# thetisproject/thetis

Measured on AMD Instinct MI355X. Metric: DG element-updates/sec, 2D SWE DG-P1 SSPRK33, higher is better.
Workload: dtype f64

## Files before the change

thetis_amd/csrc/swe2d_api_fuse.hip:

```cpp
#include "swe2d_handle.h"
#include "swe2d_fuse.h"
#include "swe2d_tiles.h"

#include <type_traits>

namespace swe2d_impl {

namespace {
template <bool... B, class F> auto pick_instance(F f) { return f(std::bool_constant<B>{}...); }
template <bool... B, class F, class... Rest> auto pick_instance(F f, bool b, Rest... rest)
{
    return b ? pick_instance<B..., true>(f, rest...) : pick_instance<B..., false>(f, rest...);
}

const TileSpec kPairTiles{3, 1, SWE_FUSE_WG, SWE_FUSE_INNER, SWE_FUSE_RING, SWE_FUSE_MAX_OUT, false};
const TileSpec kQuadPairTiles{4, 1, SWE_FUSE_WG, SWE_QFUSE_INNER, SWE_QFUSE_RING, SWE_QFUSE_MAX_OUT, false};
const TileSpec kTripleTiles{3, 2, SWE_FUSE_WG, SWE_FUSE_WG, -1, SWE_FUSE3_MAX_OUT, true};

int build_table(Handle *h, const TileSpec &spec, const std::vector<int> &order, const std::vector<unsigned char> &start, TileTable &t)
{
    const int n = h->n_cells;
    std::string err;
    if (build_tiles(h->h_nbr.data(), h->stride, n, (int)order.size() == n ? order.data() : nullptr,
                    (int)start.size() == n ? start.data() : nullptr, spec, t, err))
        return fail(h, SWE2D_ERR_UNSUPPORTED, err);
    return SWE2D_OK;
}

std::vector<int> tile_records(const TileTable &t, int nfacets)
{
    std::vector<int> rec;
    for (size_t i = 0; i < t.cell.size(); i++) {
        const unsigned *w = &t.facet[i*nfacets];
        rec.push_back(t.cell[i]);
        rec.push_back((int)(w[0] | (w[1] << SWE_FUSE_FBITS) | (w[2] << (2*SWE_FUSE_FBITS))));
        if (nfacets == 4) { rec.push_back((int)w[3]); rec.push_back(0); }
    }
    return rec;
}

int upload_tiles(Handle *h, TileSet &ts, const std::vector<int> &rec, const std::vector<int> &counts, const TileTable &t)
{
    HIP_TRY(h, hipMalloc(&ts.tile, rec.size()*sizeof(int)));
    HIP_TRY(h, hipMalloc(&ts.counts, counts.size()*sizeof(int)));
    HIP_TRY(h, hipMemcpy(ts.tile, rec.data(), rec.size()*sizeof(int), hipMemcpyHostToDevice));
    HIP_TRY(h, hipMemcpy(ts.counts, counts.data(), counts.size()*sizeof(int), hipMemcpyHostToDevice));
    ts.n_tiles = (int)t.n_inner.size();
    ts.ring[0] = t.ring[0]; ts.ring[1] = t.ring[1];
    return SWE2D_OK;
}
}

void free_tiles(TileSet &ts)
{
    if (ts.tile) (void)hipFree(ts.tile);
    if (ts.counts) (void)hipFree(ts.counts);
    ts = TileSet();
}

int fuse12_build(Handle *h)
{
    TileSet &ts = pair_tiles(h);
    if (ts.tile || h->fuse_state == -1 || stream_capturing(h)) return SWE2D_OK;
    TileTable t;
    if (int rc = build_table(h, h->npc == 4 ? kQuadPairTiles : kPairTiles, h->fuse_order, {}, t)) return rc;
    if (!fuse12_tiles_pay(h, (int)t.n_inner.size())) { h->fuse_state = -1; return SWE2D_OK; }
    return upload_tiles(h, ts, tile_records(t, h->npc), t.n_inner, t);
}

template <class Args>
static int launch_pair(Handle *h, void (*kern)(const Args), int cell_end)
{
    const TileSet &ts = pair_tiles(h);
    if (!ts.tile) return fail(h, SWE2D_ERR_UNSUPPORTED, "fused stage pair: no tile tables");
    Args q;
    fill_stage_args(h, q.st, 0, 0, 2, 0.0, 1.0, kBeta[0], 0, h->n_owned);
    q.st.idxc = h->opt[SWE2D_OPT_COMPACT_IDX] == 0 ? nullptr : h->idxc;
    q.tile = static_cast<decltype(q.tile)>(ts.tile);
    q.n_inner = ts.counts;
    q.n_tiles = ts.n_tiles;
    q.cell_end = cell_end;
    q.beta1 = kBeta[0];
    q.a0_2 = kAlpha0[1]; q.a1_2 = kAlphaIn[1]; q.beta2 = kBeta[1];
    q.out = h->state[2];
    const int grid = ((ts.n_tiles + 7)/8)*8;
    SWE_CHK_SYNC(h->stream);
    hipLaunchKernelGGL(kern, dim3(grid), dim3(SWE_FUSE_WG), 0, h->stream, q);
    HIP_TRY(h, hipGetLastError());
    stage_written(h, false, true);
    return SWE2D_OK;
}

int launch_fuse12(Handle *h, int cell_end)
{
    const bool nl = h->par.use_nonlinear_equations != 0, lf = h->par.use_lax_friedrichs_velocity != 0;
    if (h->npc == 4)
        return launch_pair(h, pick_instance([](auto a, auto b, auto c, auto d) -> void (*)(const SweFuseQuadArgs) {
                               return swe_fuse12_quad_kernel<a.value, b.value, c.value, d.value>; }, nl, lf, has_sources(h), h->affine), cell_end);
    return launch_pair(h, pick_instance([](auto a, auto b, auto c) -> void (*)(const SweFuseArgs) {
                           return swe_fuse12_kernel<a.value, b.value, c.value>; }, nl, lf, has_sources(h)), cell_end);
}

int fuse123_build(Handle *h)
{
    if (h->fuse3.tile || stream_capturing(h)) return SWE2D_OK;
    TileTable t;
    if (int rc = build_table(h, kTripleTiles, (int)h->fuse3_order.size() == h->n_cells ? h->fuse3_order : h->fuse_order, h->fuse3_start, t)) return rc;
    std::vector<int> counts;
    for (size_t i = 0; i < t.n_inner.size(); i++) { counts.push_back(t.n_inner[i]); counts.push_back(t.n_mid[i] | (t.rot[i] << 16)); }
    return upload_tiles(h, h->fuse3, tile_records(t, 3), counts, t);
}

int launch_fuse123(Handle *h, int cell_end)
{
    if (int rc = capture_parity_check(h)) return rc;
    if (int rc = fuse123_build(h)) return rc;
    if (!h->fuse3.tile) return fail(h, SWE2D_ERR_UNSUPPORTED, "fused stages: no tile tables (not built inside a stream capture)");
    SweFuse3Args q;
    fill_stage_args(h, q.st, 0, 0, 1, 0.0, 1.0, kBeta[0], 0, h->n_owned);
    q.st.idxc = h->opt[SWE2D_OPT_COMPACT_IDX] == 0 ? nullptr : h->idxc;
    q.tile = static_cast<const int2 *>(h->fuse3.tile);
    q.counts = reinterpret_cast<const int2 *>(h->fuse3.counts);
    q.n_tiles = h->fuse3.n_tiles;
    q.cell_end = cell_end;
    for (int s = 0; s < 3; s++) { q.a0[s] = s ? kAlpha0[s] : 0.0; q.a1[s] = s ? kAlphaIn[s] : 1.0; q.beta[s] = kBeta[s]; }
    q.out = h->state[1];
    auto kern = pick_instance([](auto a, auto b, auto c) -> void (*)(const SweFuse3Args) { return swe_fuse123_kernel<a.value, b.value, c.value>; },
                              h->par.use_nonlinear_equations != 0, h->par.use_lax_friedrichs_velocity != 0, has_sources(h));
    const int grid = ((h->fuse3.n_tiles + 7)/8)*8;
    SWE_CHK_SYNC(h->stream);
    hipLaunchKernelGGL(kern, dim3(grid), dim3(SWE_FUSE_WG), 0, h->stream, q);
    HIP_TRY(h, hipGetLastError());
    swap_state_buffers(h);
    unsigned long long id = 0;
    if (stream_capturing(h, &id)) {
        if (id != h->capture_id) { h->capture_id = id; h->capture_swaps = 0; }
        h->capture_swaps++;
    }
    return SWE2D_OK;
}

int capture_parity_check(Handle *h)
{
    if (h->capture_swaps == 0 && h->capture_odd == 0) return SWE2D_OK;
    unsigned long long id = 0;
    const bool capturing = stream_capturing(h, &id);
    if (h->capture_swaps) {
        if (capturing && id == h->capture_id) return SWE2D_OK;
        if (h->capture_swaps & 1) { swap_state_buffers(h); h->capture_odd++; }
        h->capture_swaps = 0;
    }
    if (capturing || h->capture_odd == 0) return SWE2D_OK;
    const int odd = h->capture_odd;
    h->capture_odd = 0;
    return fail(h, SWE2D_ERR_UNSUPPORTED, std::to_string(odd) + " stream capture(s) recorded an odd number of swe2d_solve_step_cells launches: "
                "such a graph ends on the other state buffer than it began on and cannot be replayed (the state is the one from before the "
                "capture); capture an even number per sequence");
}

}

static int checked_tile_order(Handle *h, const int32_t *cells, std::vector<int> &order)
{
    std::vector<char> seen((size_t)h->n_cells, 0);
    for (int i = 0; cells && i < h->n_cells; i++) {
        if (cells[i] < 0 || cells[i] >= h->n_cells || seen[cells[i]]) return fail(h, SWE2D_ERR_INVALID_ARGUMENT, "fused stages: the tile order is not a permutation of the cells");
        seen[cells[i]] = 1;
    }
    if (cells) order.assign(cells, cells + h->n_cells);
    return SWE2D_OK;
}

extern "C" {

int swe2d_fused_set_order(swe2d_handle *hh, const int32_t *cells_in_tile_order)
{
    Handle *h = H(hh);
    if (!h) return SWE2D_ERR_INVALID_ARGUMENT;
    HIP_TRY(h, hipSetDevice(h->device));
    std::vector<int> order;
    if (int rc = checked_tile_order(h, cells_in_tile_order, order)) return rc;
    HIP_TRY(h, hipStreamSynchronize(h->stream));
    for (TileSet *ts : {&h->fuse, &h->fuseq, &h->fuse3}) free_tiles(*ts);
    if (h->fuse_state == -1) h->fuse_state = 0;
    h->fuse_order.swap(order);
    return SWE2D_OK;
}

int swe2d_fused_set_triple_tiles(swe2d_handle *hh, const int32_t *cells_in_tile_order, const int32_t *tile_starts, int32_t n_starts)
{
    Handle *h = H(hh);
    if (!h) return SWE2D_ERR_INVALID_ARGUMENT;
    HIP_TRY(h, hipSetDevice(h->device));
    std::vector<int> order;
    std::vector<unsigned char> start;
    if (int rc = checked_tile_order(h, cells_in_tile_order, order)) return rc;
    if (n_starts < 0 || (n_starts > 0 && !tile_starts)) return fail(h, SWE2D_ERR_INVALID_ARGUMENT, "fused stages: tile starts");
    if (n_starts > 0) {
        start.assign((size_t)h->n_cells, 0);
        for (int i = 0; i < n_starts; i++) {
            if (tile_starts[i] < 0 || tile_starts[i] >= h->n_cells) return fail(h, SWE2D_ERR_INVALID_ARGUMENT, "fused stages: a tile start outside the cells");
            start[tile_starts[i]] = 1;
        }
    }
    HIP_TRY(h, hipStreamSynchronize(h->stream));
// ... 50 lines not shown
```

thetis_amd/csrc/swe2d_flow.h:

```cpp
#pragma once
#include "swe2d_kernels.h"
#include "swe2d_p2p.h"

#ifndef SWE_FLOW_OCCUPANCY
#define SWE_FLOW_OCCUPANCY __attribute__((amdgpu_waves_per_eu(2, 2)))
#endif
#define SWE_FLOW_MAX_STAGES 384
#define SWE_FLOW_MAX_CYCLES 64
#ifndef SWE_FLOW_FLAG_STRIDE
#define SWE_FLOW_FLAG_STRIDE 16
#endif
#define SWE_FLOW_SLOT_BYTES 128
#define SWE_FLOW_DIV6(t_) ((int)(((unsigned)(t_)*43691u) >> 18))
#ifndef SWE_FLOW_POLL_SLEEP
#define SWE_FLOW_POLL_SLEEP 2
#endif
#ifndef SWE_FLOW_NTR_SRC
#define SWE_FLOW_NTR_SRC 3
#endif
#ifndef SWE_FLOW_WALLFAST_SRC
#define SWE_FLOW_WALLFAST_SRC true
#endif
#ifndef SWE_FLOW_RX
#define SWE_FLOW_RX 3
// ... 37 lines not shown
    const int4 *xo4;
    const int2 *xo2;
    const int2 *xblk;
    const int *xsrc;
    void *ex;
    unsigned parity_bytes;
    int n_blocks;
    int n_stages;
    int cell_end[SWE_FLOW_MAX_STAGES];
    double a0[3], a1[3], beta[3];
    unsigned long long timeout_ticks;
    int n_cycles, stages_per_cycle;
    const int2 *xsend;
    const int *xrecv;
    unsigned *xtick;
    SweP2pCounters *xctr;
    int x_n_peers;
    int x_off[SWE_P2P_MAX_PEERS];
    void *x_rdata[SWE_P2P_MAX_PEERS];
    unsigned x_rbytes[SWE_P2P_MAX_PEERS];
    unsigned x_rslot[SWE_P2P_MAX_PEERS];
    void *x_zone;
    unsigned x_zbytes, x_slot;
    unsigned long long x_timeout;
};

__device__ __forceinline__ unsigned swe_flow_check_word(unsigned lo, unsigned hi, unsigned tag) { return tag ^ lo ^ hi; }
#ifdef SWE_FLOW_TEAR
__device__ int swe_flow_tear[4] = {-1, 0, 1, 0};
__device__ __forceinline__ void swe_flow_put_torn(__amdgpu_buffer_rsrc_t r, unsigned off, swe_u32x4 g, int aux_sys, int ticks)
{
    const swe_u32x2 hi2 = {g.z, g.w}, lo2 = {g.x, g.y};
    if (aux_sys) __builtin_amdgcn_raw_buffer_store_b64(hi2, r, off + 8u, 0, 17); else __builtin_amdgcn_raw_buffer_store_b64(hi2, r, off + 8u, 0, 16);
    asm volatile("s_waitcnt vmcnt(0)" ::: "memory");
    const unsigned long long t0 = wall_clock64();
    while (wall_clock64() - t0 < (unsigned long long)ticks) __builtin_amdgcn_s_sleep(16);
    if (aux_sys) __builtin_amdgcn_raw_buffer_store_b64(lo2, r, off, 0, 17); else __builtin_amdgcn_raw_buffer_store_b64(lo2, r, off, 0, 16);
}
#define SWE_FLOW_TORN(lb_, pc_, sys_) ((swe_flow_tear[0] == (lb_) || swe_flow_tear[0] == -2) && swe_flow_tear[1] > 0 \
                                       && ((pc_) % (swe_flow_tear[2] < 1 ? 1 : swe_flow_tear[2])) == 0 && (!(sys_) || swe_flow_tear[3]))
#endif
__device__ __forceinline__ void swe_flow_put(__amdgpu_buffer_rsrc_t r, unsigned off, double x, unsigned tag, bool torn = false)
{
    const swe_u32x2 xb = __builtin_bit_cast(swe_u32x2, x);
    const swe_u32x4 g = {xb.x, xb.y, tag, swe_flow_check_word(xb.x, xb.y, tag)};
#ifdef SWE_FLOW_TEAR
    if (torn) { swe_flow_put_torn(r, off, g, 0, swe_flow_tear[1]); return; }
#endif
    (void)torn;
    __builtin_amdgcn_raw_buffer_store_b128(g, r, off, 0, 16);
}
__device__ __forceinline__ swe_u32x4 swe_flow_get(__amdgpu_buffer_rsrc_t r, unsigned off)
{
    return __builtin_amdgcn_raw_buffer_load_b128(r, off, 0, 16);
}
__device__ __forceinline__ void swe_flow_put_sys(__amdgpu_buffer_rsrc_t r, unsigned off, double x, unsigned tag, bool torn = false)
{
    const swe_u32x2 xb = __builtin_bit_cast(swe_u32x2, x);
    const swe_u32x4 g = {xb.x, xb.y, tag, swe_flow_check_word(xb.x, xb.y, tag)};
#ifdef SWE_FLOW_TEAR
    if (torn) { swe_flow_put_torn(r, off, g, 1, swe_flow_tear[1]); return; }
#endif
    (void)torn;
    __builtin_amdgcn_raw_buffer_store_b128(g, r, off, 0, 17);
}
__device__ __forceinline__ swe_u32x4 swe_flow_get_sys(__amdgpu_buffer_rsrc_t r, unsigned off)
{
    return __builtin_amdgcn_raw_buffer_load_b128(r, off, 0, 17);
}
__device__ __forceinline__ double swe_flow_val(swe_u32x4 g)
{
    const swe_u32x2 xb = {g.x, g.y};
    return __builtin_bit_cast(double, xb);
}
__device__ __forceinline__ bool swe_flow_arrived(swe_u32x4 g, unsigned need)
{
#ifdef SWE_FLOW_NOCHECK
    return (int)(g.z - need) >= 0;
#else
    return (int)(g.z - need) >= 0 && g.w == swe_flow_check_word(g.x, g.y, g.z);
#endif
}

template <bool NONLIN, bool LF, bool SRC, int NTR, bool WD = false, int XG = SWE_FLOW_XG, int PLANE = SWE_BLOCK, int NLDS = SWE_FLOW_LDS_DOUBLES,
          int GEOM = SWE_GEOM_COMPUTE>
__device__ __forceinline__ void swe_flow_rhs_facets(const SweStageArgs &p, int k, const double u[3], const double v[3], const double e[3],
                                                    const double h[3], const double *lds, const unsigned tr[3][NTR], int bmarkers,
                                                    const double nx[3], const double ny[3], double twoA, double bu[3], double bv[3],
                                                    double be[3], const double *Dn = nullptr, const double *al = nullptr, double *geo = nullptr)
{
#pragma clang fp contract(off)
#pragma unroll
    for (int f = 0; f < 3; f++) {
        const int a = f, b = (f + 1) % 3;
        const unsigned ab0 = tr[f][0] & 0xffffu, aa0 = tr[f][0] >> 16;
        const unsigned step = ab0 >= (unsigned)XG ? 1u : (unsigned)(3*PLANE);
        const unsigned ab1 = NTR == 3 ? tr[f][NTR - 2] & 0xffffu : ab0 + step, aa1 = NTR == 3 ? tr[f][NTR - 2] >> 16 : aa0 + step;
        const unsigned ab2 = NTR == 3 ? tr[f][NTR - 1] & 0xffffu : ab0 + 2u*step, aa2 = NTR == 3 ? tr[f][NTR - 1] >> 16 : aa0 + 2u*step;
        const double unb = lds[SWE_LDSI(ab0, NLDS)], una = lds[SWE_LDSI(aa0, NLDS)];
        const double vnb = lds[SWE_LDSI(ab1, NLDS)], vna = lds[SWE_LDSI(aa1, NLDS)];
        const double enb = lds[SWE_LDSI(ab2, NLDS)], ena = lds[SWE_LDSI(aa2, NLDS)];
        double Lf, rLf;
        if constexpr (GEOM == SWE_GEOM_STORED) { Lf = geo[f*PLANE]; rLf = geo[(3 + f)*PLANE]; }
        else swe_tri_facet_len(nx[f], ny[f], Lf, rLf);
        if constexpr (GEOM == SWE_GEOM_KEEP) { geo[f*PLANE] = Lf; geo[(3 + f)*PLANE] = rLf; }
        swe_tri_facet<NONLIN, LF, WD>(p.g, p.sigma_lf, ((bmarkers >> (8*f)) & 0xff) != 0, u[a], u[b], v[a], v[b], e[a], e[b], h[a], h[b],
                                      WD ? Dn[a] : 0.0, WD ? Dn[b] : 0.0, WD ? al[a] : 0.0, WD ? al[b] : 0.0, una, unb, vna, vnb, ena, enb,
                                      nx[f], ny[f], Lf, rLf, bu[a], bu[b], bv[a], bv[b], be[a], be[b]);
    }
    if (SRC) {
        double H[3], gxs[3], gys[3];
        swe_tri_depths<NONLIN, WD>(h, e, Dn, H);
        swe_tri_grad(nx, ny, gxs, gys);
        swe_source_terms(p, k, p.stride, twoA, u, v, H, gxs, gys, bu, bv, be);
    }
}

#ifdef SWE_WAVE_TIMING
#ifndef SWE_FLOW_TS_STAGE
#define SWE_FLOW_TS_STAGE 7
#endif
#define SWE_FT(i) do { if (s == SWE_FLOW_TS_STAGE && lane == 0 && lb < SWE_WT_MAX) swe_wave_ts[i][lb] = wall_clock64(); } while (0)
#else
#define SWE_FT(i)
#endif


template <bool NONLIN, bool LF, bool SRC, bool FX, int POLL = 6, bool WD = false>
__global__ __launch_bounds__(SWE_BLOCK) SWE_FLOW_OCCUPANCY void swe_flow_kernel(const SweFlowArgs q)
{
#pragma clang fp contract(off)
    __shared__ double lds[SWE_FLOW_LDS_DOUBLES];
    __shared__ int xsrc[SWE_FLOW_MAX_RIM];
    __shared__ int lact[SWE_BLOCK];
    __shared__ unsigned lrec[SWE_BLOCK];
    __shared__ int lpeer[SWE_BLOCK];
    __shared__ unsigned char lpub[SWE_FLOW_MAX_RIM];
    __shared__ double lu0[9][SWE_BLOCK];
    const SweStageArgs &p = q.st;
    const int lb = swe_logical_block(blockIdx.x, gridDim.x);
    if (lb >= q.n_blocks) return;
    const int lane = (int)threadIdx.x;
    const int kcode = q.fcell[lb*SWE_BLOCK + lane];
    const bool real = kcode >= 0;
    const int k = real ? kcode : -1 - kcode;
    const size_t S = p.stride;
    const unsigned S8 = (unsigned)S*8u;
    unsigned *const myflag = q.flag + (size_t)lb*SWE_FLOW_FLAG_STRIDE;
    const unsigned base = *myflag;
    const unsigned fin = base + (unsigned)q.n_stages;
    if (!FX && !__any(real && k < q.cell_end[0])) {
        if (lane == 0) *myflag = fin;
        return;
    }
    const unsigned k8 = (unsigned)k*8u;
    const __amdgpu_buffer_rsrc_t rex = __builtin_amdgcn_make_buffer_rsrc(q.ex, 0, 3*q.parity_bytes, 0x00020000);
    const int2 myslots = q.xblk[lb];
    const int nrim = myslots.y;
    for (int i = lane; i < nrim; i += SWE_BLOCK) xsrc[SWE_LDSI(i, SWE_FLOW_MAX_RIM)] = q.xsrc[myslots.x + i];

    int bmarkers, bkind1 = 0;
    constexpr int NTR = WD ? 1 : SWE_FLOW_NTR_SRC;
    unsigned tr[3][NTR];
    int xown[3];
    double h[3], nx[3], ny[3], al[3] = {0.0, 0.0, 0.0};
    double u[3], v[3], e[3];
    {
        const int4 q4 = p.idx4[k];
        const int2 q2 = p.idx2[k];
        const int4 x4 = q.xo4[lb*SWE_BLOCK + lane];
        const int2 x2 = q.xo2[lb*SWE_BLOCK + lane];
        const int nb[3] = {q4.x, q4.y, q4.z};
        const int vid[3] = {q4.w, q2.x, q2.y};
        const int xin[3] = {x4.w, x2.x, x2.y};
        xown[0] = x4.x; xown[1] = x4.y; xown[2] = x4.z;
        bmarkers = (nb[0] < 0 ? -nb[0] : 0) | (nb[1] < 0 ? (-nb[1]) << 8 : 0) | (nb[2] < 0 ? (-nb[2]) << 16 : 0);
        if (bmarkers != 0) {
            const int m1 = (bmarkers & 0xff) ? (bmarkers & 0xff) : ((bmarkers & 0xff00) ? ((bmarkers >> 8) & 0xff) : (bmarkers >> 16));
            bkind1 = m1 < SWE_MAX_MARKERS ? p.bc.kind[m1] : 0;
        }
        const swe_rsrc_t gu = swe_rsrc(q.buf[0]), gv = swe_rsrc(q.buf[0] + 3*S), ge = swe_rsrc(q.buf[0] + 6*S);
#pragma unroll
        for (int i = 0; i < 3; i++) {
            u[i] = swe_ld(gu, k8, i*S8);
// ... 437 lines not shown
```

thetis_amd/csrc/swe2d_fuse.h:

```cpp
#pragma once
#include "swe2d_kernels.h"
#include "swe2d_flow.h"

#ifndef SWE_FUSE_WG
#define SWE_FUSE_WG 256
#endif
#ifndef SWE_FUSE_MIN_WG
#define SWE_FUSE_MIN_WG 3
#endif
#ifndef SWE_FUSE_INNER
#define SWE_FUSE_INNER 192
#endif
#define SWE_FUSE_FBITS 10
#define SWE_FUSE_RING (SWE_FUSE_WG - SWE_FUSE_INNER)
#define SWE_FUSE_XG (9*SWE_FUSE_WG)
#define SWE_FUSE_MAX_OUT (2*SWE_FUSE_RING)
#define SWE_FUSE_LDS (SWE_FUSE_XG + 6*SWE_FUSE_MAX_OUT)

struct SweFuseArgs {
    SweStageArgs st;
    const int2 *tile;
    const int *n_inner;
    int n_tiles;
    int cell_end;
// ... 79 lines not shown
#pragma unroll
        for (int f = 0; f < 3; f++) {
            if (outside[f]) {
                const unsigned at = ((unsigned)tl.y >> (SWE_FUSE_FBITS*f)) & 0x1ffu;
#pragma unroll
                for (int j = 0; j < 6; j++) lds[SWE_LDSI(SWE_FUSE_XG + 6*at + j, SWE_FUSE_LDS)] = r0[f][j];
            }
        }
    }
    __syncthreads();
    double o1u[3], o1v[3], o1e[3];
    double twoA = 0.0;
    if (real) {
        twoA = fma(nx[0], ny[1], -(ny[0]*nx[1]));
        double bu[3], bv[3], be[3], wu[3], wv[3], we[3];
        double H[3];
        swe_tri_depths<NONLIN, false>(h, e, nullptr, H);
        swe_tri_cell<NONLIN>(p.g, u, v, e, H, nx, ny, bu, bv, be);
        swe_flow_rhs_facets<NONLIN, LF, SRC, 1, false, SWE_FUSE_XG, SWE_FUSE_WG, SWE_FUSE_LDS>(p, k, u, v, e, h, lds, tr, bmarkers, nx, ny, twoA, bu, bv, be);
#pragma unroll
        for (int i = 0; i < 3; i++) { wu[i] = 1.0*u[i]; wv[i] = 1.0*v[i]; we[i] = 1.0*e[i]; }
        swe_tri_finish<NONLIN, LF, false, true>(p, k, q.beta1, twoA, u, v, e, h, nullptr, nullptr, nx, ny, bmarkers, bkind1, bu, bv, be,
                                                wu, wv, we, true, o1u, o1v, o1e);
    }
    __syncthreads();
    if (real) {
#pragma unroll
        for (int i = 0; i < 3; i++) { lds[i*SWE_FUSE_WG + lane] = o1u[i]; lds[(3 + i)*SWE_FUSE_WG + lane] = o1v[i]; lds[(6 + i)*SWE_FUSE_WG + lane] = o1e[i]; }
    }
    const bool act2 = lane < n_inner && k < q.cell_end;
    if (act2) {
#pragma unroll
        for (int i = 0; i < 3; i++) {
            lw[i][lane] = fma(q.a0_2, u[i], q.a1_2*o1u[i]);
            lw[3 + i][lane] = fma(q.a0_2, v[i], q.a1_2*o1v[i]);
            lw[6 + i][lane] = fma(q.a0_2, e[i], q.a1_2*o1e[i]);
        }
    }
    __syncthreads();
    if (act2) {
#pragma unroll
        for (int i = 0; i < 3; i++) asm volatile("" : "+v"(nx[i]), "+v"(ny[i]), "+v"(h[i]));
#pragma unroll
        for (int f = 0; f < 3; f++) asm volatile("" : "+v"(tr[f][0]));
        asm volatile("" : "+v"(bmarkers), "+v"(twoA));
        double bu[3], bv[3], be[3], wu[3], wv[3], we[3], ou[3], ov[3], oe[3];
        double H[3];
        swe_tri_depths<NONLIN, false>(h, o1e, nullptr, H);
        swe_tri_cell<NONLIN>(p.g, o1u, o1v, o1e, H, nx, ny, bu, bv, be);
        swe_flow_rhs_facets<NONLIN, LF, SRC, 1, false, SWE_FUSE_XG, SWE_FUSE_WG, SWE_FUSE_LDS>(p, k, o1u, o1v, o1e, h, lds, tr, bmarkers, nx, ny, twoA, bu, bv, be);
#pragma unroll
        for (int i = 0; i < 3; i++) { wu[i] = lw[i][lane]; wv[i] = lw[3 + i][lane]; we[i] = lw[6 + i][lane]; }
        swe_tri_finish<NONLIN, LF, false, true>(p, k, q.beta2, twoA, o1u, o1v, o1e, h, nullptr, nullptr, nx, ny, bmarkers, bkind1, bu, bv, be,
                                                wu, wv, we, true, ou, ov, oe);
        const swe_rsrc_t gou = swe_rsrc(q.out), gov = swe_rsrc(q.out + 3*S), goe = swe_rsrc(q.out + 6*S);
#pragma unroll
        for (int i = 0; i < 3; i++) {
            swe_st(gou, k8, i*S8, ou[i]);
            swe_st(gov, k8, i*S8, ov[i]);
            swe_st(goe, k8, i*S8, oe[i]);
        }
    }
}

#ifndef SWE_FUSE3_MAX_OUT
#define SWE_FUSE3_MAX_OUT 224
#endif
#ifndef SWE_FUSE3_GEOM
#define SWE_FUSE3_GEOM 1
#endif
#define SWE_FUSE3_NGEO 7
#define SWE_FUSE3_GEO (18*SWE_FUSE_WG)
#define SWE_FUSE3_XG (SWE_FUSE3_GEOM ? 9*SWE_FUSE_WG : 18*SWE_FUSE_WG)
#define SWE_FUSE3_LDS (SWE_FUSE3_GEOM ? SWE_FUSE3_GEO + SWE_FUSE3_NGEO*SWE_FUSE_WG : SWE_FUSE3_XG + 6*SWE_FUSE3_MAX_OUT)
static_assert(6*SWE_FUSE3_MAX_OUT <= 9*SWE_FUSE_WG, "the staging area must fit P1");
#ifndef SWE_FUSE3_SRC_MIN_WG
#define SWE_FUSE3_SRC_MIN_WG 2
#endif

struct SweFuse3Args {
    SweStageArgs st;
    const int2 *tile;
    const int2 *counts;
    int n_tiles;
    int cell_end;
    double a0[3], a1[3], beta[3];
    double *out;
};

template <bool NONLIN, bool LF, bool SRC = false>
__global__ __launch_bounds__(SWE_FUSE_WG, SRC ? SWE_FUSE3_SRC_MIN_WG : SWE_FUSE_MIN_WG) void swe_fuse123_kernel(const SweFuse3Args q)
{
#pragma clang fp contract(off)
    __shared__ double lds[SWE_FUSE3_LDS];
    const SweStageArgs &p = q.st;
    const int tile = swe_logical_block(blockIdx.x, gridDim.x);
    if (tile >= q.n_tiles) return;
    const int lane = (int)threadIdx.x;
    const int2 tl = q.tile[(size_t)tile*SWE_FUSE_WG + lane];
    const bool real = tl.x >= 0;
    const int k = real ? tl.x : 0;
    const int2 cnt = q.counts[tile];
    const int n_inner = cnt.x, n_mid = cnt.y & 0xffff, rot64 = (cnt.y >> 16) << 6;
    const size_t S = p.stride;
    const unsigned S8 = (unsigned)S*8u, k8 = (unsigned)k*8u;
    double *const P1 = lds + 9*SWE_FUSE_WG;
#ifdef SWE_WAVE_TIMING
    int wt_bodies = __any(real) ? 1 : 0;
#endif

    int bmarkers = 0, bkind1 = 0;
    unsigned tr[3][1];
    double h[3], nx[3], ny[3], u[3], v[3], e[3];
    if (real) {
        int nb[3], vid[3];
        swe_conn_load(p.idxc, p.idx4, p.idx2, k, nb, vid);
        bmarkers = (nb[0] < 0 ? -nb[0] : 0) | (nb[1] < 0 ? (-nb[1]) << 8 : 0) | (nb[2] < 0 ? (-nb[2]) << 16 : 0);
        if (bmarkers != 0) {
            const int m1 = (bmarkers & 0xff) ? (bmarkers & 0xff) : ((bmarkers & 0xff00) ? ((bmarkers >> 8) & 0xff) : (bmarkers >> 16));
            bkind1 = m1 < SWE_MAX_MARKERS ? p.bc.kind[m1] : 0;
        }
        const swe_rsrc_t gu = swe_rsrc(p.uin), gv = swe_rsrc(p.uin + 3*S), ge = swe_rsrc(p.uin + 6*S);
#pragma unroll
        for (int i = 0; i < 3; i++) {
            u[i] = swe_ld(gu, k8, i*S8);
            v[i] = swe_ld(gv, k8, i*S8);
            e[i] = swe_ld(ge, k8, i*S8);
        }
        double r0[3][6];
        bool outside[3];
#pragma unroll
        for (int f = 0; f < 3; f++) {
            const int nbf = nb[f];
            const unsigned w = ((unsigned)tl.y >> (SWE_FUSE_FBITS*f)) & 0x3ffu;
            outside[f] = (w & 0x200u) != 0u;
            const unsigned at = w & 0x1ffu;
            const int f2 = nbf >= 0 ? (nbf & 3) : f, f2a = f2 == 2 ? 0 : f2 + 1;
            {
                const unsigned ab = outside[f] ? (unsigned)(SWE_FUSE3_XG + 6*at) : (unsigned)(f2*SWE_FUSE_WG + at);
                const unsigned aa = outside[f] ? (unsigned)(SWE_FUSE3_XG + 6*at + 3) : (unsigned)(f2a*SWE_FUSE_WG + at);
                tr[f][0] = ab | (aa << 16);
            }
            const int code = outside[f] ? nbf : ((k << 2) | f);
            const unsigned kn8 = (unsigned)(code >> 2)*8u;
            const int g2 = code & 3;
            const unsigned ob = kn8 + (g2 == 0 ? 0u : (g2 == 1 ? S8 : 2u*S8));
            const unsigned oa = kn8 + (g2 == 0 ? S8 : (g2 == 1 ? 2u*S8 : 0u));
            r0[f][0] = swe_ld(gu, ob, 0); r0[f][1] = swe_ld(gv, ob, 0); r0[f][2] = swe_ld(ge, ob, 0);
            r0[f][3] = swe_ld(gu, oa, 0); r0[f][4] = swe_ld(gv, oa, 0); r0[f][5] = swe_ld(ge, oa, 0);
        }
        double px[3], py[3];
        const swe_rsrc_t rvx = swe_rsrc(p.vx), rvy = swe_rsrc(p.vy), rvh = swe_rsrc(p.vh);
#pragma unroll
        for (int i = 0; i < 3; i++) {
            const unsigned v8 = (unsigned)vid[i]*8u;
            px[i] = swe_ld(rvx, v8, 0);
            py[i] = swe_ld(rvy, v8, 0);
            h[i] = swe_ld(rvh, v8, 0);
        }
#pragma unroll
        for (int f = 0; f < 3; f++) {
            const int b = (f + 1) % 3;
            nx[f] = py[b] - py[f];
            ny[f] = px[f] - px[b];
        }
#pragma unroll
        for (int i = 0; i < 3; i++) { lds[i*SWE_FUSE_WG + lane] = u[i]; lds[(3 + i)*SWE_FUSE_WG + lane] = v[i]; lds[(6 + i)*SWE_FUSE_WG + lane] = e[i]; }
#pragma unroll
        for (int f = 0; f < 3; f++) {
            if (outside[f]) {
                const unsigned at = ((unsigned)tl.y >> (SWE_FUSE_FBITS*f)) & 0x1ffu;
#pragma unroll
                for (int j = 0; j < 6; j++) lds[SWE_LDSI(SWE_FUSE3_XG + 6*at + j, SWE_FUSE3_LDS)] = r0[f][j];
            }
        }
    }
    __syncthreads();
    constexpr int GEOM1 = SWE_FUSE3_GEOM ? SWE_GEOM_KEEP : SWE_GEOM_COMPUTE, GEOM23 = SWE_FUSE3_GEOM ? SWE_GEOM_STORED : SWE_GEOM_COMPUTE;
    double twoA = 0.0;
    double *const G = lds + SWE_FUSE3_GEO + lane;
    if (real) {
        twoA = fma(nx[0], ny[1], -(ny[0]*nx[1]));
        double bu[3], bv[3], be[3], wu[3], wv[3], we[3], ou[3], ov[3], oe[3];
        double H[3];
        swe_tri_depths<NONLIN, false>(h, e, nullptr, H);
        swe_tri_cell<NONLIN>(p.g, u, v, e, H, nx, ny, bu, bv, be);
        swe_flow_rhs_facets<NONLIN, LF, SRC, 1, false, SWE_FUSE3_XG, SWE_FUSE_WG, SWE_FUSE3_LDS, GEOM1>(p, k, u, v, e, h, lds, tr, bmarkers, nx, ny, twoA, bu, bv, be,
                                                                                                     nullptr, nullptr, G);
#pragma unroll
        for (int i = 0; i < 3; i++) { wu[i] = 1.0*u[i]; wv[i] = 1.0*v[i]; we[i] = 1.0*e[i]; }
        swe_tri_finish<NONLIN, LF, false, true, GEOM1, SWE_FUSE_WG>(p, k, q.beta[0], twoA, u, v, e, h, nullptr, nullptr, nx, ny, bmarkers, bkind1,
                                                                    bu, bv, be, wu, wv, we, true, ou, ov, oe, G);
#pragma unroll
        for (int i = 0; i < 3; i++) { u[i] = ou[i]; v[i] = ov[i]; e[i] = oe[i]; }
    }
    if (SWE_FUSE3_GEOM) __syncthreads();
    if (real) {
#pragma unroll
        for (int i = 0; i < 3; i++) { P1[i*SWE_FUSE_WG + lane] = u[i]; P1[(3 + i)*SWE_FUSE_WG + lane] = v[i]; P1[(6 + i)*SWE_FUSE_WG + lane] = e[i]; }
    }
    __syncthreads();
#pragma unroll 1
    for (int s = 1; s < 3; s++) {
        const int role = (lane - rot64) & (SWE_FUSE_WG - 1);
        const bool act = role < (s == 1 ? n_mid : n_inner) && (s == 1 || k < q.cell_end);
#ifdef SWE_WAVE_TIMING
        wt_bodies += __any(act) ? 1 : 0;
#endif
        double ou[3], ov[3], oe[3];
        if (act) {
#pragma unroll
            for (int i = 0; i < 3; i++) asm volatile("" : "+v"(nx[i]), "+v"(ny[i]), "+v"(h[i]));
#pragma unroll
            for (int f = 0; f < 3; f++) asm volatile("" : "+v"(tr[f][0]));
            asm volatile("" : "+v"(bmarkers));
            if (SRC || !SWE_FUSE3_GEOM) asm volatile("" : "+v"(twoA));
            double bu[3], bv[3], be[3], wu[3], wv[3], we[3];
            double H[3];
            swe_tri_depths<NONLIN, false>(h, e, nullptr, H);
            swe_tri_cell<NONLIN>(p.g, u, v, e, H, nx, ny, bu, bv, be);
            swe_flow_rhs_facets<NONLIN, LF, SRC, 1, false, SWE_FUSE3_XG, SWE_FUSE_WG, 9*SWE_FUSE_WG, GEOM23>(p, k, u, v, e, h, P1, tr, bmarkers, nx, ny, twoA, bu, bv, be,
                                                                                                          nullptr, nullptr, G);
            const double a0 = q.a0[s], a1 = q.a1[s];
#pragma unroll
            for (int i = 0; i < 3; i++) {
                wu[i] = fma(a0, lds[i*SWE_FUSE_WG + lane], a1*u[i]);
                wv[i] = fma(a0, lds[(3 + i)*SWE_FUSE_WG + lane], a1*v[i]);
                we[i] = fma(a0, lds[(6 + i)*SWE_FUSE_WG + lane], a1*e[i]);
            }
            swe_tri_finish<NONLIN, LF, false, true, GEOM23, SWE_FUSE_WG>(p, k, q.beta[s], twoA, u, v, e, h, nullptr, nullptr, nx, ny, bmarkers,
                                                                         bkind1, bu, bv, be, wu, wv, we, true, ou, ov, oe, G);
        }
        if (s == 1) {
            __syncthreads();
            if (act) {
#pragma unroll
                for (int i = 0; i < 3; i++) { P1[i*SWE_FUSE_WG + lane] = ou[i]; P1[(3 + i)*SWE_FUSE_WG + lane] = ov[i]; P1[(6 + i)*SWE_FUSE_WG + lane] = oe[i]; }
#pragma unroll
                for (int i = 0; i < 3; i++) { u[i] = ou[i]; v[i] = ov[i]; e[i] = oe[i]; }
            }
            __syncthreads();
        } else if (act) {
            const swe_rsrc_t gou = swe_rsrc(q.out), gov = swe_rsrc(q.out + 3*S), goe = swe_rsrc(q.out + 6*S);
#pragma unroll
            for (int i = 0; i < 3; i++) {
                swe_st(gou, k8, i*S8, ou[i]);
                swe_st(gov, k8, i*S8, ov[i]);
                swe_st(goe, k8, i*S8, oe[i]);
            }
        }
    }
#ifdef SWE_WAVE_TIMING
    if ((lane & 63) == 0 && 4*blockIdx.x + (lane >> 6) < 6*SWE_WT_MAX) {
        unsigned hw, xcc;
        asm volatile("s_getreg_b32 %0, hwreg(HW_REG_HW_ID)" : "=s"(hw));
        asm volatile("s_getreg_b32 %0, hwreg(HW_REG_XCC_ID)" : "=s"(xcc));
        (&swe_wave_ts[0][0])[4*blockIdx.x + (lane >> 6)] = (unsigned long long)hw | ((unsigned long long)(xcc & 0xf) << 32)
                                                           | ((unsigned long long)wt_bodies << 40) | (1ull << 44);
    }
#endif
}


#define SWE_QFUSE_INNER 192
#define SWE_QFUSE_RING (SWE_FUSE_WG - SWE_QFUSE_INNER)
#define SWE_QFUSE_XG (12*SWE_FUSE_WG)
#define SWE_QFUSE_MAX_OUT (3*SWE_QFUSE_RING)
#define SWE_QFUSE_LDS (SWE_QFUSE_XG + 6*SWE_QFUSE_MAX_OUT)

struct SweFuseQuadArgs {
    SweStageArgs st;
    const int4 *tile;
    const int *n_inner;
    int n_tiles;
    int cell_end;
    double beta1, a0_2, a1_2, beta2;
    double *out;
};

template <bool NONLIN, bool LF, bool SRC, bool AFFINE>
__global__ __launch_bounds__(SWE_FUSE_WG, SWE_FUSE_MIN_WG) void swe_fuse12_quad_kernel(const SweFuseQuadArgs q)
{
#pragma clang fp contract(off)
    __shared__ double lds[SWE_QFUSE_LDS];
    __shared__ double lu0[12*SWE_QFUSE_INNER];
    const SweStageArgs &p = q.st;
    const int tile = swe_logical_block(blockIdx.x, gridDim.x);
    if (tile >= q.n_tiles) return;
    const int lane = (int)threadIdx.x;
    const int4 tl = q.tile[(size_t)tile*SWE_FUSE_WG + lane];
    const bool real = tl.x >= 0;
    const int k = real ? tl.x : 0;
    const int n_inner = q.n_inner[tile];
    const size_t S = p.stride;
    const unsigned S8 = (unsigned)S*8u, k8 = (unsigned)k*8u, S4 = (unsigned)S*4u, k4 = (unsigned)k*4u;

    unsigned tr[4] = {0u, 0u, 0u, 0u}, bmarkers = 0u;
    int nb[4] = {-1, -1, -1, -1}, vid[4] = {0, 0, 0, 0};
    double u[4], v[4], e[4];
    if (real) {
#pragma unroll
        for (int i = 0; i < 4; i++) {
            nb[i] = swe_ldi(swe_rsrc(p.nbr), k4, i*S4);
            vid[i] = swe_ldi(swe_rsrc(p.cv), k4, i*S4);
// ... 87 lines not shown
```

thetis_amd/csrc/swe2d_handle.h:

```cpp
#pragma once
#include "../../include/swe2d.h"
#include "swe2d_kernels.h"
#include "swe2d_sipg.h"
#include "swe2d_flow.h"
#include "swe2d_p2p.h"

#include <dlfcn.h>
#include <unistd.h>

#include <algorithm>
#include <cmath>
#include <cstdio>
#include <cstdlib>
#include <cstring>
#include <new>
#include <string>
#include <vector>
#include <atomic>
#include <mutex>

static_assert(SWE2D_MAX_MARKERS == SWE_MAX_MARKERS, "marker table size mismatch");
static_assert(SWE2D_MAX_FARMS == SWE_MAX_FARMS && SWE2D_MAX_THRUST_TABLE == SWE_MAX_THRUST_TABLE, "turbine farm table size mismatch");

#ifdef SWE_RANGE_CHECK
#include <map>
#include <mutex>
namespace {
std::mutex g_chk_mutex;
std::map<unsigned long long, unsigned long long> g_chk_allocs;
bool g_chk_dirty = true;
unsigned long long g_chk_launches = 0;
void swe_chk_upload_locked()
{
    static SweChkTable t;
    t.n = 0;
    for (auto &kv : g_chk_allocs) if (t.n < SWE_CHK_MAX) { t.lo[t.n] = kv.first; t.hi[t.n] = kv.second; t.n++; }
    (void)hipDeviceSynchronize();
    (void)hipMemcpyToSymbol(HIP_SYMBOL(swe_chk_tab), &t, sizeof(t));
    g_chk_dirty = false;
}
hipError_t swe_chk_malloc(void **p, size_t n)
{
    const hipError_t e = hipMalloc(p, n);
    if (e == hipSuccess && *p) {
        std::lock_guard<std::mutex> lock(g_chk_mutex);
        const char *st = getenv("THETIS_AMD_RANGE_SELFTEST");
        g_chk_allocs[(unsigned long long)*p] = (unsigned long long)*p + ((st && atoi(st)) ? n/2 : n);
        swe_chk_upload_locked();
    }
    return e;
}
template <class T> hipError_t swe_chk_malloc(T **p, size_t n) { return swe_chk_malloc((void **)p, n); }
hipError_t swe_chk_free(void *p)
{
    { std::lock_guard<std::mutex> lock(g_chk_mutex); g_chk_allocs.erase((unsigned long long)p); g_chk_dirty = true; }
    return hipFree(p);
}
void swe_chk_sync(hipStream_t stream)
{
    std::lock_guard<std::mutex> lock(g_chk_mutex);
    g_chk_launches++;
    if (!g_chk_dirty) return;
    hipStreamCaptureStatus cs = hipStreamCaptureStatusNone;
    if (stream && hipStreamIsCapturing(stream, &cs) == hipSuccess && cs != hipStreamCaptureStatusNone) return;
    swe_chk_upload_locked();
}
}
#define hipMalloc(p, n) swe_chk_malloc(p, n)
#define hipFree(p) swe_chk_free(p)
#define SWE_CHK_SYNC(stream) swe_chk_sync(stream)
extern "C" int swe2d_debug_range_report(unsigned long long out[5])
{
    std::lock_guard<std::mutex> lock(g_chk_mutex);
    (void)hipDeviceSynchronize();
    if (hipMemcpyFromSymbol(out, HIP_SYMBOL(swe_chk_report), 4*sizeof(unsigned long long)) != hipSuccess) return 1;
    out[3] = g_chk_launches;
    out[4] = g_chk_allocs.size();
    return 0;
}
#else
#define SWE_CHK_SYNC(stream) ((void)0)
#endif

namespace swe2d_impl {

extern thread_local std::string g_create_error;

extern const double kBeta[3], kAlpha0[3], kAlphaIn[3];

extern std::atomic<unsigned long long> g_next_uid;

struct TileSet {
    void *tile = nullptr;
    int *counts = nullptr;
    int n_tiles = 0;
    long long ring[2] = {0, 0};
};

struct Handle {
    unsigned long long uid = g_next_uid.fetch_add(1ull);
    int device = 0;
    hipStream_t stream = nullptr;
    bool own_stream = false;
    hipStream_t my_stream = nullptr;
    hipStream_t xstream = nullptr;
    int n_cells = 0, n_owned = 0, n_interior = 0, n_vertices = 0;
    int npc = 3;
    bool affine = true;
    bool affine_local = true;
    size_t stride = 0;
    double *state[3] = {nullptr, nullptr, nullptr};
    int *nbr = nullptr, *cv = nullptr;
    struct FacetList { std::vector<int32_t> cells, facets; int *dev = nullptr; };
    FacetList facet_lists[8];
    int facet_list_next = 0;
    int4 *opp4 = nullptr;
    int *bnd_cells = nullptr;
    int n_bnd = 0;
    int opt[SWE2D_OPT_COUNT];
    Handle() { for (int i = 0; i < SWE2D_OPT_COUNT; i++) opt[i] = -1; }
    bool stage_valid[2] = {false, false};
    int capture_swaps = 0;
    unsigned long long capture_id = 0;
    int capture_odd = 0;
    int4 *idx4 = nullptr;
    int2 *idx2 = nullptr;
    int4 *idxc = nullptr;
    TileSet fuse, fuseq, fuse3;
    int fuse_state = 0;
    std::vector<int> fuse_order;
    std::vector<int> fuse3_order;
    std::vector<unsigned char> fuse3_start;
    int n_conn_escapes = 0;
    std::vector<int> h_nbr;
    unsigned *flow_flag = nullptr, *flow_status = nullptr;
    int4 *flow_xo4 = nullptr;
    int2 *flow_xo2 = nullptr;
    int2 *flow_xblk = nullptr;
    int *flow_xsrc = nullptr;
    std::vector<int> h_send, h_recv;
    std::vector<int> flow_fpos;
    int2 *flow_xsend = nullptr;
    int *flow_xrecv = nullptr;
    unsigned *flow_xtick = nullptr;
    int flow_push_blocks = 0, flow_recv_blocks = 0;
    bool flow_x_ready = false;
    int *flow_cell = nullptr;
    unsigned flow_parity_bytes = 0;
    void *flow_ex = nullptr;
    size_t flow_ex_bytes = 0;
    int flow_blocks = 0;
    int flow_capacity = -1;
    int flow_max_rim = 0;
    int launch_parity = 0;
    bool flow_used = false;
    double *vx = nullptr, *vy = nullptr, *vh = nullptr;
    double *bc_field[4] = {nullptr, nullptr, nullptr, nullptr};
    double *valpha = nullptr;
    bool wd = false;
    bool state_holds_D = false;
    struct Snapshot { void *data = nullptr; size_t bytes = 0; bool holds_D = false; };
    Snapshot snapshot[SWE2D_SNAPSHOT_SLOTS];
    bool visc = false;
    double *nu_v = nullptr;
    double nu_const = 0.0, sipg_factor = 1.0;
    int visc_grad_div = 0, visc_grad_depth = 1;
    double *field[SWE2D_FIELD_COUNT] = {nullptr, nullptr, nullptr, nullptr, nullptr, nullptr, nullptr, nullptr, nullptr};
    double scalar[SWE2D_SCALAR_COUNT] = {-1.0, -1.0, -1.0, 0.0, -1.0};
    double *stage_uv = nullptr, *stage_eta = nullptr;
    double *partial = nullptr;
    int n_partial_blocks = 0;
    unsigned long long *diag_acc = nullptr;
    int *send_cells = nullptr, *recv_cells = nullptr;
    int n_send = 0, n_recv = 0;
    struct P2p {
        void *zone = nullptr;
        size_t zone_bytes = 0;
// ... 270 lines not shown
```

thetis_amd/csrc/swe2d_tiles.h:

```cpp
#pragma once
#include <cstddef>
#include <string>
#include <utility>
#include <vector>

#ifndef SWE_FUSE3_ROT
#define SWE_FUSE3_ROT(tile) ((int)(((unsigned)(tile)*0x9E3779B1u) >> 30))
#endif

namespace swe2d_impl {

constexpr unsigned kTileOutside = 0x200u;

struct TileSpec {
    int nfacets;
    int rings;
    int wg;
    int max_inner;
    int max_ring1;
    int max_out;
    bool rotate;
};

struct TileTable {
    std::vector<int> cell;
    std::vector<unsigned> facet;
    std::vector<int> n_inner, n_mid, rot;
    long long ring[2] = {0, 0};
};

inline int build_tiles(const int *nbr, size_t stride, int n_cells, const int *order, const unsigned char *start,
                       const TileSpec &sp, TileTable &t, std::string &err)
{
    const int n = n_cells, nf = sp.nfacets, wg = sp.wg;
    const char *who = sp.rings == 2 ? "fused stages: " : "fused stage pair: ";
    t = TileTable();
    std::vector<unsigned char> state((size_t)n, 0);
    std::vector<int> lane_of((size_t)n, -1), touched, inner;
    std::vector<std::pair<int, unsigned char>> undo;
    int count[4] = {0, 0, 0, 0};
    auto set = [&](int c, unsigned char ns) {
        undo.push_back({c, state[c]});
        if (state[c] == 0) touched.push_back(c);
        count[state[c]]--; state[c] = ns; count[ns]++;
    };
    for (int pos = 0; pos < n;) {
        inner.clear(); touched.clear();
        count[1] = count[2] = count[3] = 0;
        while (pos < n && (int)inner.size() < sp.max_inner) {
            if (start && start[pos] && !inner.empty()) break;
            const int kk = order ? order[pos] : pos;
            undo.clear();
            const size_t touched_before = touched.size();
            set(kk, 1);
            for (int f = 0; f < nf; f++) {
                const int code = nbr[(size_t)f*stride + kk];
                if (code < 0) continue;
                const int c1 = code >> 2;
                if (state[c1] == 0 || state[c1] == 3) {
                    set(c1, 2);
                    for (int g = 0; sp.rings == 2 && g < nf; g++) {
                        const int code2 = nbr[(size_t)g*stride + c1];
                        if (code2 >= 0 && state[code2 >> 2] == 0) set(code2 >> 2, 3);
                    }
                }
            }
            if (count[1] + count[2] + count[3] > wg || (sp.max_ring1 >= 0 && count[2] > sp.max_ring1) || (nf - 1)*count[sp.rings + 1] > sp.max_out) {
                if (inner.empty()) {
                    err = std::string(who) + (sp.rings == 2 ? "a cell whose two rings do not fit a tile" : "a cell with more neighbours than a ring holds");
                    return 1;
                }
                for (size_t i = undo.size(); i-- > 0;) { count[state[undo[i].first]]--; state[undo[i].first] = undo[i].second; count[undo[i].second]++; }
                touched.resize(touched_before);
                break;
            }
            inner.push_back(kk);
            pos++;
        }
        std::vector<int> cells(inner);
        for (int want = 2; want <= 3; want++)
            for (int c : touched) if (state[c] == want) cells.push_back(c);
        const int ni = (int)inner.size(), nm = ni + count[2], nt = (int)cells.size();
        if (nt != count[1] + count[2] + count[3] || ni != count[1] || nt > wg) { err = std::string(who) + "tile bookkeeping"; return 1; }
        const int tile = (int)t.n_inner.size();
        const int rot = sp.rotate ? SWE_FUSE3_ROT(tile) & 3 : 0;
        auto phys = [rot, wg](int role) { return (role + 64*rot) & (wg - 1); };
        for (int l = 0; l < nt; l++) lane_of[cells[l]] = phys(l);
        const size_t base = (size_t)tile*wg;
        t.cell.resize(base + wg, -1);
        t.facet.resize((base + wg)*nf, 0u);
        const int outermost = sp.rings == 2 ? nm : ni;
        int n_out = 0;
        for (int l = 0; l < nt; l++) {
            const int c = cells[l];
            t.cell[base + phys(l)] = c;
            for (int f = 0; f < nf; f++) {
                const int code = nbr[(size_t)f*stride + c];
                unsigned field;
                if (code < 0) field = (unsigned)phys(l);
                else if (state[code >> 2] != 0) field = (unsigned)lane_of[code >> 2];
                else {
                    if (l < outermost || n_out >= sp.max_out) { err = std::string(who) + "ring bookkeeping"; return 1; }
                    field = kTileOutside | (unsigned)n_out++;
                }
                t.facet[(base + phys(l))*nf + f] = field;
            }
        }
        t.n_inner.push_back(ni); t.n_mid.push_back(nm); t.rot.push_back(rot);
        t.ring[0] += count[2]; t.ring[1] += count[3];
        for (int c : cells) { state[c] = 0; lane_of[c] = -1; }
    }
    return 0;
}

}
```

Before: 31.57 billion.

## Spread halo-slot gathers across lanes and use byte-offset LDS facet addresses

```diff
diff --git a/thetis_amd/csrc/swe2d_api_fuse.hip b/thetis_amd/csrc/swe2d_api_fuse.hip
--- a/thetis_amd/csrc/swe2d_api_fuse.hip
+++ b/thetis_amd/csrc/swe2d_api_fuse.hip
@@ -45,6 +45,14 @@
     HIP_TRY(h, hipMalloc(&ts.counts, counts.size()*sizeof(int)));
     HIP_TRY(h, hipMemcpy(ts.tile, rec.data(), rec.size()*sizeof(int), hipMemcpyHostToDevice));
     HIP_TRY(h, hipMemcpy(ts.counts, counts.data(), counts.size()*sizeof(int), hipMemcpyHostToDevice));
+    std::vector<int> slots;
+    for (size_t i = 0; i + 1 < t.slot_first.size(); i++) { slots.push_back(t.slot_first[i]); slots.push_back(t.slot_first[i + 1] - t.slot_first[i]); }
+    std::vector<int> src(t.slot_src);
+    src.push_back(0);
+    HIP_TRY(h, hipMalloc(&ts.slots, slots.size()*sizeof(int)));
+    HIP_TRY(h, hipMalloc(&ts.slot_src, src.size()*sizeof(int)));
+    HIP_TRY(h, hipMemcpy(ts.slots, slots.data(), slots.size()*sizeof(int), hipMemcpyHostToDevice));
+    HIP_TRY(h, hipMemcpy(ts.slot_src, src.data(), src.size()*sizeof(int), hipMemcpyHostToDevice));
     ts.n_tiles = (int)t.n_inner.size();
     ts.ring[0] = t.ring[0]; ts.ring[1] = t.ring[1];
     return SWE2D_OK;
@@ -55,6 +63,8 @@
 {
     if (ts.tile) (void)hipFree(ts.tile);
     if (ts.counts) (void)hipFree(ts.counts);
+    if (ts.slots) (void)hipFree(ts.slots);
+    if (ts.slot_src) (void)hipFree(ts.slot_src);
     ts = TileSet();
 }
 
@@ -121,6 +131,8 @@
     q.st.idxc = h->opt[SWE2D_OPT_COMPACT_IDX] == 0 ? nullptr : h->idxc;
     q.tile = static_cast<const int2 *>(h->fuse3.tile);
     q.counts = reinterpret_cast<const int2 *>(h->fuse3.counts);
+    q.slots = reinterpret_cast<const int2 *>(h->fuse3.slots);
+    q.slot_src = h->fuse3.slot_src;
     q.n_tiles = h->fuse3.n_tiles;
     q.cell_end = cell_end;
     for (int s = 0; s < 3; s++) { q.a0[s] = s ? kAlpha0[s] : 0.0; q.a1[s] = s ? kAlphaIn[s] : 1.0; q.beta[s] = kBeta[s]; }
diff --git a/thetis_amd/csrc/swe2d_flow.h b/thetis_amd/csrc/swe2d_flow.h
--- a/thetis_amd/csrc/swe2d_flow.h
+++ b/thetis_amd/csrc/swe2d_flow.h
@@ -143,8 +143,16 @@
 #endif
 }
 
+#define SWE_TR_INDEX 0
+#define SWE_TR_BYTES 1
+#define SWE_TR_BYTES_INSIDE 2
+#ifdef SWE_RANGE_CHECK
+#define SWE_LDSB(p_, b_, n_) ((p_)[SWE_LDSI((b_) >> 3, n_)])
+#else
+#define SWE_LDSB(p_, b_, n_) (*reinterpret_cast<const double *>(reinterpret_cast<const char *>(p_) + (b_)))
+#endif
 template <bool NONLIN, bool LF, bool SRC, int NTR, bool WD = false, int XG = SWE_FLOW_XG, int PLANE = SWE_BLOCK, int NLDS = SWE_FLOW_LDS_DOUBLES,
-          int GEOM = SWE_GEOM_COMPUTE>
+          int GEOM = SWE_GEOM_COMPUTE, int TRB = SWE_TR_INDEX>
 __device__ __forceinline__ void swe_flow_rhs_facets(const SweStageArgs &p, int k, const double u[3], const double v[3], const double e[3],
                                                     const double h[3], const double *lds, const unsigned tr[3][NTR], int bmarkers,
                                                     const double nx[3], const double ny[3], double twoA, double bu[3], double bv[3],
@@ -155,12 +163,21 @@
     for (int f = 0; f < 3; f++) {
         const int a = f, b = (f + 1) % 3;
         const unsigned ab0 = tr[f][0] & 0xffffu, aa0 = tr[f][0] >> 16;
-        const unsigned step = ab0 >= (unsigned)XG ? 1u : (unsigned)(3*PLANE);
-        const unsigned ab1 = NTR == 3 ? tr[f][NTR - 2] & 0xffffu : ab0 + step, aa1 = NTR == 3 ? tr[f][NTR - 2] >> 16 : aa0 + step;
-        const unsigned ab2 = NTR == 3 ? tr[f][NTR - 1] & 0xffffu : ab0 + 2u*step, aa2 = NTR == 3 ? tr[f][NTR - 1] >> 16 : aa0 + 2u*step;
-        const double unb = lds[SWE_LDSI(ab0, NLDS)], una = lds[SWE_LDSI(aa0, NLDS)];
-        const double vnb = lds[SWE_LDSI(ab1, NLDS)], vna = lds[SWE_LDSI(aa1, NLDS)];
-        const double enb = lds[SWE_LDSI(ab2, NLDS)], ena = lds[SWE_LDSI(aa2, NLDS)];
+        double unb, una, vnb, vna, enb, ena;
+        if constexpr (TRB == SWE_TR_INDEX) {
+            const unsigned step = ab0 >= (unsigned)XG ? 1u : (unsigned)(3*PLANE);
+            const unsigned ab1 = NTR == 3 ? tr[f][NTR - 2] & 0xffffu : ab0 + step, aa1 = NTR == 3 ? tr[f][NTR - 2] >> 16 : aa0 + step;
+            const unsigned ab2 = NTR == 3 ? tr[f][NTR - 1] & 0xffffu : ab0 + 2u*step, aa2 = NTR == 3 ? tr[f][NTR - 1] >> 16 : aa0 + 2u*step;
+            unb = lds[SWE_LDSI(ab0, NLDS)]; una = lds[SWE_LDSI(aa0, NLDS)];
+            vnb = lds[SWE_LDSI(ab1, NLDS)]; vna = lds[SWE_LDSI(aa1, NLDS)];
+            enb = lds[SWE_LDSI(ab2, NLDS)]; ena = lds[SWE_LDSI(aa2, NLDS)];
+        } else {
+            static_assert(TRB == SWE_TR_INDEX || NTR == 1, "byte addresses: one packed word per facet");
+            const unsigned step = TRB == SWE_TR_BYTES_INSIDE ? (unsigned)(24*PLANE) : (ab0 >= (unsigned)(8*XG) ? 8u : (unsigned)(24*PLANE));
+            unb = SWE_LDSB(lds, ab0, NLDS); una = SWE_LDSB(lds, aa0, NLDS);
+            vnb = SWE_LDSB(lds, ab0 + step, NLDS); vna = SWE_LDSB(lds, aa0 + step, NLDS);
+            enb = SWE_LDSB(lds, ab0 + 2u*step, NLDS); ena = SWE_LDSB(lds, aa0 + 2u*step, NLDS);
+        }
         double Lf, rLf;
         if constexpr (GEOM == SWE_GEOM_STORED) { Lf = geo[f*PLANE]; rLf = geo[(3 + f)*PLANE]; }
         else swe_tri_facet_len(nx[f], ny[f], Lf, rLf);
diff --git a/thetis_amd/csrc/swe2d_fuse.h b/thetis_amd/csrc/swe2d_fuse.h
--- a/thetis_amd/csrc/swe2d_fuse.h
+++ b/thetis_amd/csrc/swe2d_fuse.h
@@ -185,6 +185,8 @@
     SweStageArgs st;
     const int2 *tile;
     const int2 *counts;
+    const int2 *slots;
+    const int *slot_src;
     int n_tiles;
     int cell_end;
     double a0[3], a1[3], beta[3];
@@ -211,10 +213,16 @@
 #ifdef SWE_WAVE_TIMING
     int wt_bodies = __any(real) ? 1 : 0;
 #endif
+    const int2 sl = q.slots[tile];
+    const int slot = ((lane & 63) << 2) | (lane >> 6);
+    int scode = -1;
+    if (slot < sl.y) scode = q.slot_src[sl.x + slot];
 
     int bmarkers = 0, bkind1 = 0;
     unsigned tr[3][1];
     double h[3], nx[3], ny[3], u[3], v[3], e[3];
+    double px[3], py[3];
+    const swe_rsrc_t gu = swe_rsrc(p.uin), gv = swe_rsrc(p.uin + 3*S), ge = swe_rsrc(p.uin + 6*S);
     if (real) {
         int nb[3], vid[3];
         swe_conn_load(p.idxc, p.idx4, p.idx2, k, nb, vid);
@@ -223,36 +231,23 @@
             const int m1 = (bmarkers & 0xff) ? (bmarkers & 0xff) : ((bmarkers & 0xff00) ? ((bmarkers >> 8) & 0xff) : (bmarkers >> 16));
             bkind1 = m1 < SWE_MAX_MARKERS ? p.bc.kind[m1] : 0;
         }
-        const swe_rsrc_t gu = swe_rsrc(p.uin), gv = swe_rsrc(p.uin + 3*S), ge = swe_rsrc(p.uin + 6*S);
 #pragma unroll
         for (int i = 0; i < 3; i++) {
             u[i] = swe_ld(gu, k8, i*S8);
             v[i] = swe_ld(gv, k8, i*S8);
             e[i] = swe_ld(ge, k8, i*S8);
         }
-        double r0[3][6];
-        bool outside[3];
 #pragma unroll
         for (int f = 0; f < 3; f++) {
             const int nbf = nb[f];
             const unsigned w = ((unsigned)tl.y >> (SWE_FUSE_FBITS*f)) & 0x3ffu;
-            outside[f] = (w & 0x200u) != 0u;
+            const bool outside = (w & 0x200u) != 0u;
             const unsigned at = w & 0x1ffu;
             const int f2 = nbf >= 0 ? (nbf & 3) : f, f2a = f2 == 2 ? 0 : f2 + 1;
-            {
-                const unsigned ab = outside[f] ? (unsigned)(SWE_FUSE3_XG + 6*at) : (unsigned)(f2*SWE_FUSE_WG + at);
-                const unsigned aa = outside[f] ? (unsigned)(SWE_FUSE3_XG + 6*at + 3) : (unsigned)(f2a*SWE_FUSE_WG + at);
-                tr[f][0] = ab | (aa << 16);
-            }
-            const int code = outside[f] ? nbf : ((k << 2) | f);
-            const unsigned kn8 = (unsigned)(code >> 2)*8u;
-            const int g2 = code & 3;
-            const unsigned ob = kn8 + (g2 == 0 ? 0u : (g2 == 1 ? S8 : 2u*S8));
-            const unsigned oa = kn8 + (g2 == 0 ? S8 : (g2 == 1 ? 2u*S8 : 0u));
-            r0[f][0] = swe_ld(gu, ob, 0); r0[f][1] = swe_ld(gv, ob, 0); r0[f][2] = swe_ld(ge, ob, 0);
-            r0[f][3] = swe_ld(gu, oa, 0); r0[f][4] = swe_ld(gv, oa, 0); r0[f][5] = swe_ld(ge, oa, 0);
-        }
-        double px[3], py[3];
+            const unsigned ab = outside ? (unsigned)(8*SWE_FUSE3_XG) + 48u*at : (unsigned)(8*SWE_FUSE_WG*f2) + 8u*at;
+            const unsigned aa = outside ? (unsigned)(8*SWE_FUSE3_XG + 24) + 48u*at : (unsigned)(8*SWE_FUSE_WG*f2a) + 8u*at;
+            tr[f][0] = ab | (aa << 16);
+        }
         const swe_rsrc_t rvx = swe_rsrc(p.vx), rvy = swe_rsrc(p.vy), rvh = swe_rsrc(p.vh);
 #pragma unroll
         for (int i = 0; i < 3; i++) {
@@ -261,6 +256,17 @@
             py[i] = swe_ld(rvy, v8, 0);
             h[i] = swe_ld(rvh, v8, 0);
         }
+    }
+    double r0[6];
+    if (scode >= 0) {
+        const unsigned kn8 = (unsigned)(scode >> 2)*8u;
+        const int g2 = scode & 3;
+        const unsigned ob = kn8 + (g2 == 0 ? 0u : (g2 == 1 ? S8 : 2u*S8));
+        const unsigned oa = kn8 + (g2 == 0 ? S8 : (g2 == 1 ? 2u*S8 : 0u));
+        r0[0] = swe_ld(gu, ob, 0); r0[1] = swe_ld(gv, ob, 0); r0[2] = swe_ld(ge, ob, 0);
+        r0[3] = swe_ld(gu, oa, 0); r0[4] = swe_ld(gv, oa, 0); r0[5] = swe_ld(ge, oa, 0);
+    }
+    if (real) {
 #pragma unroll
         for (int f = 0; f < 3; f++) {
             const int b = (f + 1) % 3;
@@ -269,14 +275,10 @@
         }
 #pragma unroll
         for (int i = 0; i < 3; i++) { lds[i*SWE_FUSE_WG + lane] = u[i]; lds[(3 + i)*SWE_FUSE_WG + lane] = v[i]; lds[(6 + i)*SWE_FUSE_WG + lane] = e[i]; }
-#pragma unroll
-        for (int f = 0; f < 3; f++) {
-            if (outside[f]) {
-                const unsigned at = ((unsigned)tl.y >> (SWE_FUSE_FBITS*f)) & 0x1ffu;
-#pragma unroll
-                for (int j = 0; j < 6; j++) lds[SWE_LDSI(SWE_FUSE3_XG + 6*at + j, SWE_FUSE3_LDS)] = r0[f][j];
-            }
-        }
+    }
+    if (scode >= 0) {
+#pragma unroll
+        for (int j = 0; j < 6; j++) lds[SWE_LDSI(SWE_FUSE3_XG + 6*slot + j, SWE_FUSE3_LDS)] = r0[j];
     }
     __syncthreads();
     constexpr int GEOM1 = SWE_FUSE3_GEOM ? SWE_GEOM_KEEP : SWE_GEOM_COMPUTE, GEOM23 = SWE_FUSE3_GEOM ? SWE_GEOM_STORED : SWE_GEOM_COMPUTE;
@@ -288,7 +290,7 @@
         double H[3];
         swe_tri_depths<NONLIN, false>(h, e, nullptr, H);
         swe_tri_cell<NONLIN>(p.g, u, v, e, H, nx, ny, bu, bv, be);
-        swe_flow_rhs_facets<NONLIN, LF, SRC, 1, false, SWE_FUSE3_XG, SWE_FUSE_WG, SWE_FUSE3_LDS, GEOM1>(p, k, u, v, e, h, lds, tr, bmarkers, nx, ny, twoA, bu, bv, be,
+        swe_flow_rhs_facets<NONLIN, LF, SRC, 1, false, SWE_FUSE3_XG, SWE_FUSE_WG, SWE_FUSE3_LDS, GEOM1, SWE_TR_BYTES>(p, k, u, v, e, h, lds, tr, bmarkers, nx, ny, twoA, bu, bv, be,
                                                                                                      nullptr, nullptr, G);
 #pragma unroll
         for (int i = 0; i < 3; i++) { wu[i] = 1.0*u[i]; wv[i] = 1.0*v[i]; we[i] = 1.0*e[i]; }
@@ -322,7 +324,7 @@
             double H[3];
             swe_tri_depths<NONLIN, false>(h, e, nullptr, H);
             swe_tri_cell<NONLIN>(p.g, u, v, e, H, nx, ny, bu, bv, be);
-            swe_flow_rhs_facets<NONLIN, LF, SRC, 1, false, SWE_FUSE3_XG, SWE_FUSE_WG, 9*SWE_FUSE_WG, GEOM23>(p, k, u, v, e, h, P1, tr, bmarkers, nx, ny, twoA, bu, bv, be,
+            swe_flow_rhs_facets<NONLIN, LF, SRC, 1, false, SWE_FUSE3_XG, SWE_FUSE_WG, 9*SWE_FUSE_WG, GEOM23, SWE_TR_BYTES_INSIDE>(p, k, u, v, e, h, P1, tr, bmarkers, nx, ny, twoA, bu, bv, be,
                                                                                                           nullptr, nullptr, G);
             const double a0 = q.a0[s], a1 = q.a1[s];
 #pragma unroll
diff --git a/thetis_amd/csrc/swe2d_handle.h b/thetis_amd/csrc/swe2d_handle.h
--- a/thetis_amd/csrc/swe2d_handle.h
+++ b/thetis_amd/csrc/swe2d_handle.h
@@ -93,6 +93,8 @@
 struct TileSet {
     void *tile = nullptr;
     int *counts = nullptr;
+    int *slots = nullptr;
+    int *slot_src = nullptr;
     int n_tiles = 0;
     long long ring[2] = {0, 0};
 };
diff --git a/thetis_amd/csrc/swe2d_tiles.h b/thetis_amd/csrc/swe2d_tiles.h
--- a/thetis_amd/csrc/swe2d_tiles.h
+++ b/thetis_amd/csrc/swe2d_tiles.h
@@ -27,6 +27,8 @@
     std::vector<unsigned> facet;
     std::vector<int> n_inner, n_mid, rot;
     long long ring[2] = {0, 0};
+    std::vector<int> slot_src;
+    std::vector<int> slot_first;
 };
 
 inline int build_tiles(const int *nbr, size_t stride, int n_cells, const int *order, const unsigned char *start,
@@ -39,6 +41,7 @@
     std::vector<int> lane_of((size_t)n, -1), touched, inner;
     std::vector<std::pair<int, unsigned char>> undo;
     int count[4] = {0, 0, 0, 0};
+    t.slot_first.push_back(0);
     auto set = [&](int c, unsigned char ns) {
         undo.push_back({c, state[c]});
         if (state[c] == 0) touched.push_back(c);
@@ -102,12 +105,14 @@
                 else {
                     if (l < outermost || n_out >= sp.max_out) { err = std::string(who) + "ring bookkeeping"; return 1; }
                     field = kTileOutside | (unsigned)n_out++;
+                    t.slot_src.push_back(code);
                 }
                 t.facet[(base + phys(l))*nf + f] = field;
             }
         }
         t.n_inner.push_back(ni); t.n_mid.push_back(nm); t.rot.push_back(rot);
         t.ring[0] += count[2]; t.ring[1] += count[3];
+        t.slot_first.push_back((int)t.slot_src.size());
         for (int c : cells) { state[c] = 0; lane_of[c] = -1; }
     }
     return 0;
```

After: 32.58 billion (median of 6 runs). 3.2% higher.
